# maxim2266/csvplus

Hardware: AMD Instinct MI355X
Metric: joined rows/sec (IndexOn build + chained Join, 1e8-row 3-col orders) (higher is better)
Workload: dtype u32; 1 GPU; BASELINE configs[3]: orders(1e8 x {cust_id,prod_id,qty}).Join(UniqueIndexOn customers.id 1e7).Join(UniqueIndexOn products.prod_id 1e5); rows=100000000, customers=10000000, products=100000, rows_this_rank=100000000, exchange=none (1 GPU), output=sorted positions

## Files before the change

csvplus_amd/csrc/chain.hip:

```cpp
#include <type_traits>

#include "probe_device.hpp"

namespace cph {

constexpr int kChainThreads = 256;
constexpr int kChainWaves   = kChainThreads / kWave;
constexpr int kChainRows    = 8;
constexpr int kWaveTile     = kWave * kChainRows;
constexpr int kChainTile    = kChainThreads * kChainRows;
constexpr int kChainMasks   = kChainRows * kChainWaves;
constexpr int kMaxChain     = 4;

struct ChainStepArg {
    DevCol col;
    const uint8_t* codec;
    const uint32_t* rowtab;
    const uint2* ranktab;
    int32_t positions;
    int32_t ranktab_lds;
    const uint4* hash;
    uint32_t hash_sectors;
    uint32_t hash_slice_mask;
    int32_t src;
    const uint32_t* src_perm;
    const void* codes;
    const uint32_t* perm;
    uint64_t n_index;
    int32_t codec_bytes;
    int32_t key32;
};
struct ChainArgs {
    ChainStepArg step[kMaxChain];
    uint32_t* out_rows[kMaxChain];
    int32_t nt_streams;
    int32_t reserved_;
};
struct LeanArgs {
    int32_t identity[kMaxChain];
    ArithPlan arith[kMaxChain];
};

template <int S, bool LONG, bool WIDE, bool DBG, uint32_t LEAN = 0, int R = kChainRows, bool DEP = false>
__global__ __launch_bounds__(kChainThreads) void k_chain_dense(ChainArgs a, uint64_t nprobe, uint64_t probe_base,
                                                              uint64_t ntiles, uint64_t* __restrict__ masks,
                                                              uint32_t* __restrict__ wave_counts, int dbg_flags, LeanArgs la) {
    extern __shared__ __attribute__((aligned(16))) uint8_t smem[];
    using B = std::conditional_t<WIDE, uint64_t, uint32_t>;
    using CW = std::conditional_t<WIDE, uint64_t, uint32_t>;
    const int dbg = DBG ? dbg_flags : 0;
    CodecView cv[S];
    {
        uint8_t* p = smem;
#pragma unroll
        for (int s = 0; s < S; s++) {
            if ((LEAN >> s) & 1u) continue;
            cv[s] = codec_load_to_lds(a.step[s].codec, p);
            p += a.step[s].codec_bytes;
        }
    }
    const CPH_LDS uint32_t* rank_lds[S];
    {
        uint8_t* p = smem;
#pragma unroll
        for (int s = 0; s < S; s++) p += a.step[s].codec_bytes;
        bool any = false;
#pragma unroll
        for (int s = 0; s < S; s++) {
            rank_lds[s] = nullptr;
            const int nblk = a.step[s].ranktab_lds;
            if (LEAN != 0 && nblk) {
                uint2* dst = reinterpret_cast<uint2*>(p);
                for (int i = threadIdx.x; i < 2 * nblk; i += kChainThreads) dst[i] = a.step[s].ranktab[i];
                rank_lds[s] = (const CPH_LDS uint32_t*)p;
                p += (size_t)nblk * 16;
                any = true;
            } else if (nblk) {
                uint32_t* dst = reinterpret_cast<uint32_t*>(p);
                for (int i = threadIdx.x; i < nblk; i += kChainThreads) {
                    const uint2 b0 = a.step[s].ranktab[2 * i], b1 = a.step[s].ranktab[2 * i + 1];
                    dst[3 * i] = b0.x;
                    dst[3 * i + 1] = b1.x;
                    dst[3 * i + 2] = b0.x ? b0.y : b1.y;
                }
                rank_lds[s] = (const CPH_LDS uint32_t*)p;
                p += (size_t)((nblk * 12 + 15) & ~15);
                any = true;
            }
        }
        if (any) __syncthreads();
    }
    const int lane = lane_id();
    const uint32_t wave = (uint32_t)__builtin_amdgcn_readfirstlane(wave_id());

#pragma unroll 1
    for (uint64_t tile = blockIdx.x; tile < ntiles; tile += gridDim.x) {
        uint32_t wave_matches = 0;
#pragma unroll 1
      for (int part = 0; part < kChainRows / R; part++) {
        const uint64_t wbase = tile * kChainTile + (uint64_t)wave * kWaveTile + (uint64_t)part * (R * kWave);
        const WaveRows<R> wr = wave_rows<R>(wbase, nprobe);
        uint32_t okm = wr.okm;
        WaveSpans<R, B> sp[S];
        uint64_t c0[S][R], c1[LONG ? S : 1][R];
        CW code[S][R];
        uint32_t brow[S][R];
#pragma unroll
      for (int lvl = 0; lvl < (DEP ? S : 1); lvl++) {
#pragma unroll
        for (int s = 0; s < S; s++) {
            if (DEP && s != lvl) continue;
            if ((LEAN >> s) & 1u) continue;
            if constexpr (DEP) {
                const int32_t src = a.step[s].src;
                if (src != 0) {
                    const int t = (src < 0 ? -src : src) - 1;
                    uint32_t grow[R];
#pragma unroll
                    for (int k = 0; k < R; k++) grow[k] = 0u;
#pragma unroll
                    for (int u = 0; u < S; u++)
                        if (u < s && u == t) {
#pragma unroll
                            for (int k = 0; k < R; k++) grow[k] = (okm >> k) & 1u ? brow[u][k] : 0u;
                        }
                    if (a.step[s].src_perm) {
#pragma unroll
                        for (int k = 0; k < R; k++) grow[k] = a.step[s].src_perm[grow[k]];
                    }
                    gather_spans<R, B>(a.step[s].col, grow, &sp[s]);
                    continue;
                }
            }
            if (a.nt_streams) wave_spans<R, B, false, true>(a.step[s].col, wr, &sp[s]);
            else wave_spans<R, B>(a.step[s].col, wr, &sp[s]);
        }
#pragma unroll
        for (int s = 0; s < S; s++) {
            if (DEP && s != lvl) continue;
            if ((LEAN >> s) & 1u) {
                typedef const __attribute__((address_space(1))) uint64_t* global_u64_ptr;
                const global_u64_ptr w = (global_u64_ptr)a.step[s].col.data + wr.rbase;
                if (a.nt_streams) {
#pragma unroll
                    for (int k = 0; k < R; k++) c0[s][k] = __builtin_nontemporal_load(&w[wr.rel[k]]);
                } else {
#pragma unroll
                    for (int k = 0; k < R; k++) c0[s][k] = w[wr.rel[k]];
                }
                continue;
            }
#pragma unroll
            for (int k = 0; k < R; k++) {
                c0[s][k] = a.nt_streams ? sp[s].chunk_nt(k, 0) : sp[s].chunk(k, 0);
                if constexpr (LONG) c1[s][k] = a.nt_streams ? sp[s].chunk_nt(k, 1) : sp[s].chunk(k, 1);
            }
        }
#pragma unroll
        for (int s = 0; s < S; s++) {
            if (DEP && s != lvl) continue;
            if (DBG && (dbg & 2)) {
#pragma unroll
                for (int k = 0; k < R; k++) code[s][k] = (CW)((c0[s][k] ^ (LONG ? c1[LONG ? s : 0][k] : 0ull)) & 1023);
            } else if ((LEAN >> s) & 1u) {
                encode_rows_arith<R, CW>(la.arith[s], c0[s], code[s], &okm);
            } else if (!WIDE || cv[s].hdr->lutw_bits == 32) {
                encode_rows<R, uint32_t, B, CW, LONG>(cv[s], sp[s], c0[s], c1[LONG ? s : 0], code[s], &okm,
                                                               a.step[s].col.fixed_width != 0 && (int)a.step[s].col.fixed_width == cv[s].hdr->col_maxlen[0]);
            } else {
                encode_rows<R, uint64_t, B, CW, LONG>(cv[s], sp[s], c0[s], c1[LONG ? s : 0], code[s], &okm,
                                                               a.step[s].col.fixed_width != 0 && (int)a.step[s].col.fixed_width == cv[s].hdr->col_maxlen[0]);
            }
        }
#pragma unroll
        for (int s = 0; s < S; s++) {
            if (DEP && s != lvl) continue;
            const ChainStepArg& st = a.step[s];
            if constexpr (LEAN != 0) {
                if (la.identity[s]) {
#pragma unroll
                    for (int k = 0; k < R; k++)
                        brow[s][k] = ((okm >> k) & 1u) && (uint32_t)code[s][k] < (uint32_t)st.n_index ? (uint32_t)code[s][k] : kTableAbsent;
                } else if (rank_lds[s]) {
#pragma unroll
                    for (int k = 0; k < R; k++) {
                        const uint32_t cidx = (okm >> k) & 1u ? (uint32_t)code[s][k] : 0u;
                        const CPH_LDS uint32_t* e = rank_lds[s] + 2u * (cidx >> 5);
                        const uint32_t bits = e[0], before = e[1], bit = cidx & 31u;
                        brow[s][k] = (bits >> bit) & 1u ? before + (uint32_t)__popc(bits & ((1u << bit) - 1u)) : kTableAbsent;
                    }
                } else {
                    uint2 blk[R];
#pragma unroll
                    for (int k = 0; k < R; k++) {
                        const uint32_t cidx = (okm >> k) & 1u ? (uint32_t)code[s][k] : 0u;
                        blk[k] = st.ranktab[cidx >> 5];
                    }
#pragma unroll
                    for (int k = 0; k < R; k++) {
                        const uint32_t bit = (uint32_t)code[s][k] & 31u;
                        brow[s][k] = (blk[k].x >> bit) & 1u ? blk[k].y + (uint32_t)__popc(blk[k].x & ((1u << bit) - 1u)) : kTableAbsent;
                    }
                }
            } else if (st.ranktab) {
                if (rank_lds[s]) {
#pragma unroll
                    for (int k = 0; k < R; k++) {
                        const CW cidx = (okm >> k) & 1u ? code[s][k] : (CW)0;
                        const CPH_LDS uint32_t* e = rank_lds[s] + 3u * (uint32_t)((uint64_t)cidx >> 6);
                        const uint32_t bit = (uint32_t)cidx & 63u;
                        const uint64_t bits = (uint64_t)e[0] | ((uint64_t)e[1] << 32);
                        const bool present = (bits >> bit) & 1ull;
                        brow[s][k] = present ? e[2] + (uint32_t)__popcll(bits & ((1ull << bit) - 1ull)) : kTableAbsent;
                    }
                } else {
                    uint2 blk[R];
#pragma unroll
                    for (int k = 0; k < R; k++) {
                        const CW cidx = (okm >> k) & 1u ? code[s][k] : (CW)0;
                        blk[k] = (DBG && (dbg & 1)) ? make_uint2(~0u, 0u) : st.ranktab[(uint64_t)cidx >> 5];
                    }
#pragma unroll
                    for (int k = 0; k < R; k++) {
                        const uint32_t bit = (uint32_t)code[s][k] & 31u;
                        const bool present = (blk[k].x >> bit) & 1u;
                        brow[s][k] = present ? blk[k].y + (uint32_t)__popc(blk[k].x & ((1u << bit) - 1u)) : kTableAbsent;
                    }
                }
            } else if (st.rowtab) {
#pragma unroll
                for (int k = 0; k < R; k++) {
                    const CW cidx = (okm >> k) & 1u ? code[s][k] : (CW)0;
                    brow[s][k] = (DBG && (dbg & 1)) ? 0u : st.rowtab[cidx];
                }
            } else if (st.hash) {
                const HashView hv{st.hash, st.hash_sectors, st.hash_slice_mask};
#pragma unroll
                for (int g = 0; g < R; g += 4) {
// ... 23 lines not shown
                    uint64_t lo;
                    bool hit;
                    if (st.key32) {
                        const uint32_t* cd = reinterpret_cast<const uint32_t*>(st.codes);
                        lo = lower_bound_dev<uint32_t>(cd, 0, st.n_index, (uint32_t)code[s][k]);
                        hit = lo < st.n_index && cd[lo] == (uint32_t)code[s][k];
                    } else {
                        const uint64_t* cd = reinterpret_cast<const uint64_t*>(st.codes);
                        lo = lower_bound_dev<uint64_t>(cd, 0, st.n_index, (uint64_t)code[s][k]);
                        hit = lo < st.n_index && cd[lo] == (uint64_t)code[s][k];
                    }
                    if (hit) brow[s][k] = st.positions ? (uint32_t)lo : st.perm[lo];
                }
            }
        }
#pragma unroll
        for (int s = 0; s < S; s++) {
            if (DEP && s != lvl) continue;
#pragma unroll
            for (int k = 0; k < R; k++)
                if (brow[s][k] == kTableAbsent) okm &= ~(1u << k);
        }
      }
        const uint64_t mword = (tile * kChainWaves + wave) * kChainRows + (uint64_t)part * R;
#pragma unroll
        for (int k = 0; k < R; k++) {
            const bool ok = (okm >> k) & 1u;
            const uint64_t bal = __ballot(ok);
            wave_matches += (uint32_t)__popcll(bal);
            if (lane == 0) masks[mword + k] = bal;
            if (ok && !(DBG && (dbg & 4))) {
#pragma unroll
                for (int s = 0; s < S; s++) {
                    if (a.nt_streams) __builtin_nontemporal_store(brow[s][k], a.out_rows[s] + wr.rbase + wr.rel[k]);
                    else (a.out_rows[s] + wr.rbase)[wr.rel[k]] = brow[s][k];
                }
            }
        }
      }
        if (lane == 0) wave_counts[tile * kChainWaves + wave] = wave_matches;
    }
}

struct CodeStepArg {
    const uint32_t* codes;
    const uint32_t* rowtab;
    const uint2* ranktab;
    uint64_t n_index, table_entries;
    int32_t identity;
    int32_t reserved_;
};
struct CodeArgs {
    CodeStepArg step[kMaxChain];
    uint32_t* out_rows[kMaxChain];
};
template <int S>
__global__ __launch_bounds__(kChainThreads) void k_chain_codes(CodeArgs a, uint64_t nprobe, uint64_t ntiles, uint64_t* __restrict__ masks,
                                                              uint32_t* __restrict__ wave_counts) {
    const int lane = lane_id();
    const uint32_t wave = (uint32_t)__builtin_amdgcn_readfirstlane(wave_id());
#pragma unroll 1
    for (uint64_t tile = blockIdx.x; tile < ntiles; tile += gridDim.x) {
        const uint64_t wbase = tile * kChainTile + (uint64_t)wave * kWaveTile;
        const WaveRows<kChainRows> wr = wave_rows<kChainRows>(wbase, nprobe);
        uint32_t okm = wr.okm;
        uint32_t code[S][kChainRows], brow[S][kChainRows];
#pragma unroll
// ... 265 lines not shown
    __shared__ uint32_t s_tmp[kPjThreads / kWave + 1];
    const uint64_t i0 = (uint64_t)blockIdx.x * kPjTile + (uint64_t)threadIdx.x * kPjItems;
    uint32_t keep = 0, mine = 0;
#pragma unroll
    for (int k = 0; k < kPjItems; k++)
        if (i0 + k < n && v[i0 + k] != kTableAbsent) {
            keep |= 1u << k;
            mine++;
        }
    uint32_t total;
    uint32_t run = block_exclusive_sum<uint32_t, kPjThreads>(mine, s_tmp, &total);
    uint64_t o = (uint64_t)tile_base[blockIdx.x] + run;
#pragma unroll
    for (int k = 0; k < kPjItems; k++) {
        if (!((keep >> k) & 1u)) continue;
        a.dst64[o] = a.src64[i0 + k];
        for (int j = 0; j < a.n32; j++) a.dst32[j][o] = a.src32[j][i0 + k];
        o++;
    }
}

bool chain_fast_path_ok(const ChainStep* steps, int nsteps) {
    if (nsteps > kMaxChain) return false;
    for (int s = 0; s < nsteps; s++) {
        const cph_index* ix = steps[s].index;
        if (steps[s].ncols != 1 || ix->nkeycols != 1) return false;
        if (ix->first_dup != UINT64_MAX) return false;
        if (ix->codec.nwords != 1 || ix->codec.npos == 0 || !ix->windows.empty()) return false;
        if (codec_premultiplied_bits(ix->codec) == 0) return false;
    }
    return true;
}

template <int S>
static Status enqueue_dense(cph_ctx* ctx, const ChainStep* steps, uint64_t nprobe, uint64_t probe_base,
                            uint32_t* const* d_rows, uint64_t* d_masks, uint32_t* d_counts, uint64_t* d_total,
                            ChainArgs* args_out, unsigned* grid_out, bool positions, uint64_t* host_total = nullptr,
                            const char* prof_name = "k_chain_dense") {
    const uint64_t ntiles = (nprobe + kChainTile - 1) / kChainTile;
    ChainArgs args{};
    LeanArgs largs{};
    size_t lds = 0, rank_lds_bytes = 0;
    const int dbg = ctx->chain_debug;
    bool long_keys = false, wide = false, dep = false;
    for (int s = 0; s < S; s++) dep |= steps[s].source != 0;
    if (dep) long_keys = wide = true;
    for (int s = 0; s < S; s++) {
        const cph_index* ix = steps[s].index;
        const DevCol& c = steps[s].cols[0];
        long_keys |= ix->codec.col_maxlen[0] > 8;
        wide |= codec_premultiplied_bits(ix->codec) != 32 || !ix->codec.key32;
        wide |= !col_is_narrow(c);
    }
    uint32_t lean = 0;
    bool ident[kMaxChain] = {false, false, false, false};
    if (positions)
        for (int s = 0; s < S; s++) {
            const cph_index* ix = steps[s].index;
            ident[s] = ctx->chain_identity && ix->table_entries != 0 && ix->table_entries == ix->nrows &&
                       ix->first_dup == UINT64_MAX && ix->windows.empty();
        }
    if (positions && ctx->chain_arith && !long_keys && !wide && !dbg) {
        bool all_ranked = true;
        for (int s = 0; s < S; s++) {
            const cph_index* ix = steps[s].index;
            const DevCol& c = steps[s].cols[0];
            ArithPlan ap;
            codec_arith_plan(ix->codec, &ap);
            if (ap.enabled && ap.keylen == 8 && c.fixed_width == 8 && ((uintptr_t)c.data & 7u) == 0) lean |= 1u << s;
            if (!ident[s]) {
                CPH_TRY(index_ensure_ranktab(ctx, ix));
                all_ranked &= (bool)ix->ranktab;
            }
        }
        if (!all_ranked) lean = 0;
    }
    if (S > 2 && lean != (1u << S) - 1u) lean = 0;
    if (!lean)
        for (int s = 0; s < S; s++) ident[s] = false;
    for (int s = 0; s < S; s++)
        if (!((lean >> s) & 1u)) lds += steps[s].index->codec_dev.bytes();
    for (int s = 0; s < S; s++) {
        const cph_index* ix = steps[s].index;
        ChainStepArg& st = args.step[s];
        st.col = steps[s].cols[0];
        st.codec = ix->codec_dev.as<uint8_t>();
        st.codec_bytes = (int32_t)ix->codec_dev.bytes();
        if ((lean >> s) & 1u) {
            codec_arith_plan(ix->codec, &largs.arith[s]);
            st.codec_bytes = 0;
        }
        st.positions = positions ? 1 : 0;
        st.rowtab = nullptr;
        st.ranktab = nullptr;
        largs.identity[s] = ident[s] ? 1 : 0;
        if (ident[s]) {
        } else if (positions) {
            CPH_TRY(index_ensure_ranktab(ctx, ix));
            st.ranktab = ix->ranktab ? ix->ranktab.as<uint2>() : nullptr;
            const size_t nblk = ranktab_blocks(ix->table_entries) / 2, rb = lean ? nblk * 16 : (nblk * 12 + 15) & ~(size_t)15;
            if (st.ranktab && ctx->chain_rank_lds && lds + rank_lds_bytes + rb <= 52 * 1024) {
                st.ranktab_lds = (int32_t)nblk;
                rank_lds_bytes += rb;
            }
        } else {
            CPH_TRY(index_ensure_rowtab(ctx, ix));
            st.rowtab = ix->rowtab ? ix->rowtab.as<uint32_t>() : nullptr;
        }
        st.src = steps[s].source;
        st.src_perm = (steps[s].source > 0 && positions) ? steps[steps[s].source - 1].index->perm.as<uint32_t>() : nullptr;
        st.hash = nullptr;
        st.hash_sectors = 0;
        st.hash_slice_mask = 0;
        if (!st.rowtab && !st.ranktab && !ident[s] && index_wants_hash(ix)) {
            CPH_TRY(index_ensure_hash(ctx, ix));
            if (ix->hash_mode == kHashK1) {
                st.hash = ix->hash.as<uint4>();
                st.hash_sectors = ix->hash_sectors;
                st.hash_slice_mask = ix->hash_slice_mask;
            }
        }
        st.codes = ix->sorted_codes.get();
        st.perm = ix->perm.as<uint32_t>();
        st.n_index = ix->nrows;
        st.key32 = ix->codec.key32 ? 1 : 0;
        args.out_rows[s] = d_rows[s];
    }
    lds += rank_lds_bytes;
    args.nt_streams = ctx->chain_nt_streams == 1 || (ctx->chain_nt_streams == 2 && positions) ? 1 : 0;
    const uint64_t ncounts = ntiles * kChainWaves;
    using KernelFn = void (*)(ChainArgs, uint64_t, uint64_t, uint64_t, uint64_t*, uint32_t*, int, LeanArgs);
    static const KernelFn variants[2][2][2] = {
        {{&k_chain_dense<S, false, false, false>, &k_chain_dense<S, false, false, true>},
         {&k_chain_dense<S, false, true, false>, &k_chain_dense<S, false, true, true>}},
        {{&k_chain_dense<S, true, false, false>, &k_chain_dense<S, true, false, true>},
         {&k_chain_dense<S, true, true, false>, &k_chain_dense<S, true, true, true>}}};
    KernelFn kernel = variants[long_keys ? 1 : 0][wide ? 1 : 0][(dbg && !dep) ? 1 : 0];
    if (!dbg && ctx->chain_rows4 != 0 && ((S == 2 && long_keys && wide) || (S >= 3 && (long_keys || wide)) || S == 4 || ctx->chain_rows4 == 2)) {
        static const KernelFn r4[2][2] = {{&k_chain_dense<S, false, false, false, 0u, 4>, &k_chain_dense<S, false, true, false, 0u, 4>},
                                          {&k_chain_dense<S, true, false, false, 0u, 4>, &k_chain_dense<S, true, true, false, 0u, 4>}};
        kernel = r4[long_keys ? 1 : 0][wide ? 1 : 0];
    }
    if constexpr (S >= 2) {
        if (dep) kernel = &k_chain_dense<S, true, true, false, 0u, 4, true>;
    }
    if (lean) {
        constexpr uint32_t kAll = (1u << S) - 1u;
        if (lean == kAll) kernel = &k_chain_dense<S, false, false, false, kAll>;
        if constexpr (S == 2) {
            if (lean == 1u) kernel = &k_chain_dense<S, false, false, false, 1u>;
            if (lean == 2u) kernel = &k_chain_dense<S, false, false, false, 2u>;
        }
    }
    int per_cu = 1, cus = 256;
    CPH_TRY(kernel_setup(ctx, reinterpret_cast<const void*>(kernel), kChainThreads, lds, &per_cu));
    CPH_TRY(device_cus(ctx, &cus));
    const unsigned grid = (unsigned)std::min<uint64_t>(ntiles, (uint64_t)cus * (uint64_t)per_cu);
    {
        ProfScope ps(ctx, prof_name, 0);
        hipLaunchKernelGGL(kernel, dim3(grid), dim3(kChainThreads), lds, ctx->stream, args, nprobe, probe_base,
                           ntiles, d_masks, d_counts, dep ? 0 : dbg, largs);
    }
    if (host_total) {
        DevBuf& acc = ctx->self_clean[ctx->stream_slot].sum;
        CPH_TRY(self_clean_block(ctx, &acc, 16));
        ProfScope ps(ctx, "k_sum_counts", 4.0 * (double)ncounts);
        const unsigned sgrid = sum_counts_grid(ncounts);
        hipLaunchKernelGGL(k_sum_counts_report, dim3(sgrid), dim3(256), 0, ctx->stream, d_counts, ncounts, acc.as<unsigned long long>(),
                           reinterpret_cast<unsigned long long*>(host_total));
    } else if (d_total) {
        ProfScope ps(ctx, "k_sum_counts", 4.0 * (double)ncounts);
        CPH_HIP_TRY(hipMemsetAsync(d_total, 0, sizeof(uint64_t), ctx->stream));
        const unsigned sgrid = (unsigned)std::min<uint64_t>((ncounts + 255) / 256, 512);
        hipLaunchKernelGGL(k_sum_counts, dim3(sgrid), dim3(256), 0, ctx->stream, d_counts, ncounts,
                           reinterpret_cast<unsigned long long*>(d_total));
    }
    CPH_HIP_TRY(hipGetLastError());
    if (args_out) *args_out = args;
    if (grid_out) *grid_out = grid;
    return {};
}

bool chain_fast_path_ok(const ChainStep* steps, int nsteps);

Status chain_enqueue_dense(cph_ctx* ctx, const ChainStep* steps, int nsteps, uint64_t nprobe, uint64_t probe_base,
                           uint32_t* const* d_rows, uint64_t* d_masks, uint32_t* d_counts, uint64_t* d_total, bool positions) {
// ... 368 lines not shown
```

csvplus_amd/csrc/codec_device.hpp:

```cpp
#pragma once

#include "cph_internal.hpp"
#include "device_utils.hpp"

namespace cph {

__device__ __forceinline__ uint64_t find_first_byte(const uint8_t* data, uint64_t begin, uint64_t len, uint32_t d) {
    const uint64_t dv = 0x0101010101010101ull * (uint64_t)(d & 0xFFu);
    for (uint64_t j = 0; 8 * j < len; j++) {
        const uint64_t x = load_value_chunk(data, begin, len, (int)j) ^ dv;
        const uint64_t t = (x - 0x0101010101010101ull) & ~x & 0x8080808080808080ull;
        if (t) {
            const uint64_t pos = 8 * j + (uint64_t)((__ffsll((long long)t) - 1) >> 3);
            return pos < len ? pos : len;
        }
    }
    return len;
}

__device__ __forceinline__ void value_span_whole(const DevCol& col, uint64_t row, uint64_t* begin, uint64_t* len);
__device__ __forceinline__ void value_span(const DevCol& col, uint64_t row, uint64_t* begin, uint64_t* len) {
    value_span_whole(col, row, begin, len);
    if (col.split) {
        const uint64_t b = *begin, l = *len;
// ... 135 lines not shown
        const uint32_t sym = (uint32_t)q < len ? ((uint32_t)(chunk >> (8 * (q & 7))) & 0xFFu) + 1u : 0u;
        const W v = lutw[q * kLutStride + sym];
        bad |= v;
        acc += v;
    }
    *code = (uint64_t)acc;
    return len <= (uint32_t)maxlen && !(bad >> (sizeof(W) * 8 - 1));
}

template <int R>
struct WaveRows {
    uint64_t rbase;
    uint32_t nvalid;
    uint32_t rel[R];
    uint32_t okm;
};
template <int R>
__device__ __forceinline__ WaveRows<R> wave_rows(uint64_t wbase, uint64_t nrows ) {
    WaveRows<R> w;
    const uint64_t left = nrows > wbase ? nrows - wbase : 0;
    w.nvalid = left > (uint64_t)(R * kWave) ? (uint32_t)(R * kWave) : (uint32_t)left;
    w.rbase = w.nvalid ? wbase : nrows - 1;
    const uint32_t rmax = w.nvalid ? w.nvalid - 1 : 0;
    w.okm = 0;
    const uint32_t lane = (uint32_t)lane_id();
#pragma unroll
    for (int k = 0; k < R; k++) {
        const uint32_t r = (uint32_t)k * kWave + lane;
        w.okm |= (r < w.nvalid ? 1u : 0u) << k;
        w.rel[k] = r < rmax ? r : rmax;
    }
    return w;
}

template <int R, class B>
struct WaveSpans {
    const uint8_t* base8;
    uint32_t delta;
    B x[R];
    uint32_t len[R];
    __device__ __forceinline__ uint64_t chunk(int k, uint32_t j) const {
        return load_chunk_nobranch<B>(base8, delta, x[k], len[k], j);
    }
    __device__ __forceinline__ uint64_t chunk_nt(int k, uint32_t j) const {
        return load_chunk_nobranch<B, true>(base8, delta, x[k], len[k], j);
    }
};
template <int R, class B, bool SEG = false, bool NT = false>
__device__ __forceinline__ void wave_spans(const DevCol& c, const WaveRows<R>& wr, WaveSpans<R, B>* sp);
template <int R, class B, bool NT = false>
__device__ __forceinline__ void wave_spans_whole(const DevCol& c, const WaveRows<R>& wr, WaveSpans<R, B>* sp);
template <int R, class B, bool SEG, bool NT>
__device__ __forceinline__ void wave_spans(const DevCol& c, const WaveRows<R>& wr, WaveSpans<R, B>* sp) {
    wave_spans_whole<R, B, NT>(c, wr, sp);
    if constexpr (SEG) {
#pragma unroll
        for (int k = 0; k < R; k++) {
            const uint32_t s = sp->len[k] < c.skip ? sp->len[k] : c.skip;
            sp->x[k] += (B)s;
            uint32_t l = sp->len[k] - s;
            if (c.take != 0xFFFFFFFFu && l > c.take) l = c.take;
            sp->len[k] = l;
        }
    }
}
template <int R, class B, bool NT>
// ... 134 lines not shown
        const int qn = maxlen - 8 * j < 8 ? maxlen - 8 * j : 8;
        const CPH_LDS W* lp = lutw + (8 * j) * kLutStride;
        if (fixed) {
#pragma unroll
            for (int b = 0; b < 8; b++)
                if (b < qn) encode_position<R, W, B, true>(lp, b, (uint32_t)(8 * j + b), sp, cur, acc, bad);
        } else {
#pragma unroll
            for (int b = 0; b < 8; b++)
                if (b < qn) encode_position<R, W, B, false>(lp, b, (uint32_t)(8 * j + b), sp, cur, acc, bad);
        }
    }
    uint32_t m = *okmask;
#pragma unroll
    for (int k = 0; k < R; k++) {
        code[k] = (CW)acc[k];
        const W flag = sizeof(W) == 4 ? acc[k] : bad[k];
        const bool good = sp.len[k] <= (uint32_t)maxlen && !(flag >> (sizeof(W) * 8 - 1));
        if (!good) m &= ~(1u << k);
    }
    *okmask = m;
}

struct ArithPlan {
    uint32_t enabled;
    uint32_t mul24;
    uint32_t keylen;
    uint32_t keep[2];
    uint32_t lo[2];
    uint32_t rngc[2];
    uint32_t wa[2], wb[2];
    uint32_t ma[2];
    uint32_t s1;
};

void codec_arith_plan(const CodecHost& codec, ArithPlan* ap);

template <int R, class CW>
__device__ __forceinline__ void encode_rows_arith(const ArithPlan& ap, const uint64_t (&c0)[R], CW (&code)[R], uint32_t* okmask) {
    uint32_t m = *okmask;
    uint32_t zl[R], zh[R];
#pragma unroll
    for (int k = 0; k < R; k++) {
        const uint32_t xl = (uint32_t)c0[k], xh = (uint32_t)(c0[k] >> 32);
        zl[k] = xl - ap.lo[0];
        zh[k] = xh - ap.lo[1];
        const uint32_t tl = zl[k] + ap.rngc[0], th = zh[k] + ap.rngc[1];
        const uint32_t bad = ((xl | zl[k] | tl) | (xh | zh[k] | th)) & 0x80808080u;
        if (bad) m &= ~(1u << k);
    }
    if (ap.mul24) {
#pragma unroll
        for (int k = 0; k < R; k++) {
            const uint32_t pa0 = __builtin_amdgcn_udot4(zl[k], ap.wa[0], 0u, false);
            const uint32_t pa1 = __builtin_amdgcn_udot4(zh[k], ap.wa[1], 0u, false);
            const uint32_t w0 = __builtin_amdgcn_udot4(zl[k], ap.wb[0], __umul24(pa0, ap.ma[0]), false);
            code[k] = (CW)__builtin_amdgcn_udot4(zh[k], ap.wb[1], __umul24(pa1, ap.ma[1]) + __umul24(w0, ap.s1), false);
        }
    } else {
#pragma unroll
        for (int k = 0; k < R; k++) {
            const uint32_t pa0 = __builtin_amdgcn_udot4(zl[k], ap.wa[0], 0u, false);
            const uint32_t pa1 = __builtin_amdgcn_udot4(zh[k], ap.wa[1], 0u, false);
            const uint32_t w0 = __builtin_amdgcn_udot4(zl[k], ap.wb[0], pa0 * ap.ma[0], false);
            code[k] = (CW)__builtin_amdgcn_udot4(zh[k], ap.wb[1], pa1 * ap.ma[1] + w0 * ap.s1, false);
        }
    }
    *okmask = m;
}

template <bool LONGV = true>
struct ValueHeadT {
    uint64_t begin = 0, len = 0, c0 = 0, c1 = 0, c2 = 0;
    __device__ __forceinline__ void span(const DevCol& col, uint64_t row) { value_span(col, row, &begin, &len); }
    __device__ __forceinline__ void chunks(const DevCol& col) {
        c0 = len > 0 ? load_value_chunk(col.data, begin, len, 0) : 0;
        c1 = len > 8 ? load_value_chunk(col.data, begin, len, 1) : 0;
        c2 = len > 16 ? load_value_chunk(col.data, begin, len, 2) : 0;
    }
    __device__ __forceinline__ void chunks_nobranch(const DevCol& col) {
        const uint64_t p = (uint64_t)(uintptr_t)col.data;
        const uint8_t* base8 = (const uint8_t*)(uintptr_t)(p & ~7ull);
        const uint32_t delta = (uint32_t)(p & 7ull);
        const uint32_t l32 = len > 0xFFFFFFFFull ? 0xFFFFFFFFu : (uint32_t)len;
        const uint64_t a = load_chunk_nobranch<uint64_t>(base8, delta, begin, l32, 0);
        const uint64_t b = load_chunk_nobranch<uint64_t>(base8, delta, begin, l32, 1);
        const uint64_t c = load_chunk_nobranch<uint64_t>(base8, delta, begin, l32, 2);
        c0 = l32 > 0 ? a : 0;
        c1 = l32 > 8 ? b : 0;
        c2 = l32 > 16 ? c : 0;
    }
    __device__ __forceinline__ void load(const DevCol& col, uint64_t row) {
        span(col, row);
        chunks(col);
    }
    __device__ __forceinline__ uint64_t chunk(const DevCol& col, int j) const {
        if constexpr (LONGV) {
            if (8ull * (uint64_t)j >= len) return 0;
            return j == 0 ? c0 : j == 1 ? c1 : j == 2 ? c2 : load_value_chunk(col.data, begin, len, j);
// ... 146 lines not shown
```

csvplus_amd/csrc/keycodec.hip:

```cpp
#include <algorithm>
#include <cmath>
#include <mutex>

#include "codec_device.hpp"
#include "host_encode_kernels.hpp"

namespace cph {

constexpr int kStatsThreads = 256;
constexpr int kStatsRows = 8;

template <class B, bool SEG>
__global__ __launch_bounds__(kStatsThreads) void k_col_stats(DevCol col, uint32_t* __restrict__ g_minmax,
                                                            uint32_t* __restrict__ g_mask) {
    __shared__ __attribute__((aligned(16))) uint8_t s_flag[kMaxKeyBytes * 256];
    __shared__ uint32_t s_min, s_max;
    {
        uint4* z = reinterpret_cast<uint4*>(s_flag);
        for (int i = threadIdx.x; i < kMaxKeyBytes * 256 / 16; i += kStatsThreads) z[i] = make_uint4(0, 0, 0, 0);
    }
    if (threadIdx.x == 0) { s_min = 0xFFFFFFFFu; s_max = 0; }
    __syncthreads();

    uint32_t mn = 0xFFFFFFFFu, mx = 0;
// ... 1597 lines not shown
                    else { dtags[k][h] = tag; dicts[k][h] = key; g.count++; }
                }
            }
        }
    }, 2048);
    const int best = split_pick(ctx, 0, cand, hs, step, most, plain_bits);
    if (best < 0) return {};
    const SplitStats& st = hs[(size_t)best];
    if (st.flags || st.count == 0 || st.count > (uint32_t)kWideDictMax || st.pmax > (uint32_t)kWideBytes || st.smax > (uint32_t)kSplitMaxSuffix ||
        st.vmax > (uint32_t)kSplitMaxValue)
        return {};
    std::vector<WideKey> dict;
    for (size_t s2 = 0; s2 < dtags[(size_t)best].size(); s2++)
        if (dtags[(size_t)best][s2]) dict.push_back(dicts[(size_t)best][s2]);
    if (dict.size() != st.count) return {};
    CodecHost trial;
    bool usable = false;
    CPH_TRY(split_assemble(ctx, 0, 1, nullptr, (uint32_t)cand[(size_t)best], st, &dict, plain_bits, &trial, &usable));
    if (!usable) return {};
    trial.spec_checked = true;
    if (trial.nwords != 1 || !trial.key32 || trial.word_states[0] > (1ull << 27)) return {};
    if (codec_sort_cost(trial) < bits_sort_cost(plain_bits)) *codec = std::move(trial);
    return {};
}

int codec_premultiplied_bits(const CodecHost& cd) {
    if (cd.nwords != 1 || cd.npos <= 0 || cd.has_groups()) return 0;
    const int bits = cd.word_states[0] <= (1ull << 31) ? 32 : 64;
    return (size_t)cd.npos * kLutStride * (size_t)(bits / 8) <= 48 * 1024 ? bits : 0;
}

void codec_arith_plan(const CodecHost& cd, ArithPlan* ap) {
    *ap = ArithPlan{};
    if (cd.ncols != 1 || cd.nwords != 1 || cd.has_groups() || cd.npos < 1 || cd.npos > 8) return;
    if (cd.col_minlen[0] != cd.col_maxlen[0] || cd.word_states[0] > (1ull << 31)) return;
    uint32_t lo[8] = {0}, rng[8] = {0}, radix[8] = {1, 1, 1, 1, 1, 1, 1, 1};
    for (int p = 0; p < cd.npos; p++) {
        const uint16_t* lut = &cd.lut[(size_t)p * kLutStride];
        if (lut[0] != kLutInvalid) return;
        int first = -1, last = -1, count = 0;
        for (int b = 0; b < 256; b++)
            if (lut[1 + b] != kLutInvalid) { if (first < 0) first = b; last = b; count++; }
        if (first < 0 || last >= 0x80 || last - first + 1 != count || count > 255 || count != (int)cd.radix[(size_t)p]) return;
        for (int b = first; b <= last; b++)
            if (lut[1 + b] != (uint16_t)(b - first)) return;
        lo[p] = (uint32_t)first;
        rng[p] = (uint32_t)(last - first);
        radix[p] = (uint32_t)count;
    }
    ap->keylen = (uint32_t)cd.npos;
    for (int w = 0; w < 2; w++) {
        for (int i = 0; i < 4; i++) {
            const int p = 4 * w + i;
            if (p < cd.npos) ap->keep[w] |= 0xFFu << (8 * i);
            ap->lo[w] |= lo[p] << (8 * i);
            ap->rngc[w] |= (0x7Fu - rng[p]) << (8 * i);
        }
        ap->wa[w] = radix[4 * w + 1] | 1u << 8;
        ap->wb[w] = radix[4 * w + 3] << 16 | 1u << 24;
        ap->ma[w] = radix[4 * w + 2] * radix[4 * w + 3];
    }
    const uint64_t s0 = (uint64_t)radix[0] * radix[1] * radix[2] * radix[3];
    const uint64_t s1 = (uint64_t)radix[4] * radix[5] * radix[6] * radix[7];
    ap->s1 = (uint32_t)s1;
    ap->mul24 = s0 <= (1ull << 24) && s1 < (1ull << 24) ? 1u : 0u;
    ap->enabled = 1;
}

Status codec_upload(cph_ctx* ctx, const CodecHost& cd, DevBuf* dev) {
    CodecDevHeader h{};
    h.ncols = cd.ncols;
    h.npos = cd.npos;
    h.nwords = cd.nwords;
    h.key32 = cd.key32 ? 1 : 0;
    for (int c = 0; c <= cd.ncols; c++) h.col_start[c] = cd.col_start[c];
    for (int c = cd.ncols + 1; c <= kMaxKeyCols; c++) h.col_start[c] = cd.npos;
    for (int c = 0; c < cd.ncols; c++) h.col_maxlen[c] = cd.col_maxlen[c];
    auto align16 = [](size_t x) { return (x + 15) & ~(size_t)15; };
    size_t off = align16(sizeof(CodecDevHeader));
    h.mult_off = (int32_t)off;
    off = align16(off + sizeof(uint64_t) * (size_t)cd.npos);
    h.wordof_off = (int32_t)off;
    off = align16(off + (size_t)cd.npos + 1);
    const int lutw_bits = codec_premultiplied_bits(cd);
    h.lutw_bits = lutw_bits;
    if (lutw_bits) {
        h.lut_off = 0;
        h.lutw_off = (int32_t)off;
        off = align16(off + (size_t)(lutw_bits / 8) * (size_t)cd.npos * kLutStride);
    } else {
        h.lutw_off = 0;
        h.lut_off = (int32_t)off;
        off = align16(off + sizeof(uint16_t) * (size_t)cd.npos * kLutStride);
    }
    if (cd.has_groups()) {
        h.ngroups = 0;
        for (int p = 0; p < cd.npos; p++) h.ngroups += cd.unit[(size_t)p] == kUnitHead || cd.unit[(size_t)p] == kUnitWide;
        h.unit_off = (int32_t)off;
        off = align16(off + (size_t)cd.npos);
// ... 584 lines not shown
```

Baseline: 149.0 billion rows/s.

## Add variable-length arithmetic lean path and compile-time switches for chain join kernel

```diff
diff --git a/csvplus_amd/csrc/chain.hip b/csvplus_amd/csrc/chain.hip
--- a/csvplus_amd/csrc/chain.hip
+++ b/csvplus_amd/csrc/chain.hip
@@ -41,13 +41,18 @@
     ArithPlan arith[kMaxChain];
 };
 
-template <int S, bool LONG, bool WIDE, bool DBG, uint32_t LEAN = 0, int R = kChainRows, bool DEP = false>
-__global__ __launch_bounds__(kChainThreads) void k_chain_dense(ChainArgs a, uint64_t nprobe, uint64_t probe_base,
+constexpr int kSwNt = 1, kSwMul24 = 2, kSwRuntime = 4;
+constexpr int chain_min_waves(int S, uint32_t lean) { return S <= 2 && lean == (1u << S) - 1u ? 4 : 1; }
+template <int S, bool LONG, bool WIDE, bool DBG, uint32_t LEAN = 0, int R = kChainRows, bool DEP = false, uint32_t VAR = 0, int SW = kSwRuntime>
+__global__ __launch_bounds__(kChainThreads, chain_min_waves(S, LEAN)) void k_chain_dense(ChainArgs a, uint64_t nprobe, uint64_t probe_base,
                                                               uint64_t ntiles, uint64_t* __restrict__ masks,
                                                               uint32_t* __restrict__ wave_counts, int dbg_flags, LeanArgs la) {
     extern __shared__ __attribute__((aligned(16))) uint8_t smem[];
     using B = std::conditional_t<WIDE, uint64_t, uint32_t>;
     using CW = std::conditional_t<WIDE, uint64_t, uint32_t>;
+    static_assert((VAR & ~LEAN) == 0 && (LEAN != 0 || SW == kSwRuntime), "VAR and SW describe lean steps");
+    constexpr int kM24 = (SW & kSwRuntime) ? -1 : ((SW & kSwMul24) ? 1 : 0);
+    const bool nt_streams = (SW & kSwRuntime) ? a.nt_streams != 0 : (SW & kSwNt) != 0;
     const int dbg = DBG ? dbg_flags : 0;
     CodecView cv[S];
     {
@@ -60,6 +65,7 @@
         }
     }
     const CPH_LDS uint32_t* rank_lds[S];
+    bool rank_in_lds[S];
     {
         uint8_t* p = smem;
 #pragma unroll
@@ -68,6 +74,7 @@
 #pragma unroll
         for (int s = 0; s < S; s++) {
             rank_lds[s] = nullptr;
+            rank_in_lds[s] = a.step[s].ranktab_lds != 0;
             const int nblk = a.step[s].ranktab_lds;
             if (LEAN != 0 && nblk) {
                 uint2* dst = reinterpret_cast<uint2*>(p);
@@ -92,6 +99,15 @@
     }
     const int lane = lane_id();
     const uint32_t wave = (uint32_t)__builtin_amdgcn_readfirstlane(wave_id());
+    uint64_t vend[S];
+#pragma unroll
+    for (int s = 0; s < S; s++) {
+        vend[s] = 0;
+        if ((VAR >> s) & 1u) {
+            const DevCol& c = a.step[s].col;
+            vend[s] = c.fixed_width ? nprobe * (uint64_t)c.fixed_width : (uint64_t)reinterpret_cast<const uint32_t*>(c.offsets)[nprobe];
+        }
+    }
 
 #pragma unroll 1
     for (uint64_t tile = blockIdx.x; tile < ntiles; tile += gridDim.x) {
@@ -99,17 +115,44 @@
 #pragma unroll 1
       for (int part = 0; part < kChainRows / R; part++) {
         const uint64_t wbase = tile * kChainTile + (uint64_t)wave * kWaveTile + (uint64_t)part * (R * kWave);
-        const WaveRows<R> wr = wave_rows<R>(wbase, nprobe);
+        const WaveRows<R> wr = LEAN != 0 ? wave_rows_full_first<R>(wbase, nprobe) : wave_rows<R>(wbase, nprobe);
         uint32_t okm = wr.okm;
         WaveSpans<R, B> sp[S];
         uint64_t c0[S][R], c1[LONG ? S : 1][R];
         CW code[S][R];
         uint32_t brow[S][R];
+        uint32_t vbeg[VAR ? S : 1][R], vstop[VAR ? S : 1][R], vlen[VAR ? S : 1][R];
+        uint64_t vbase[VAR ? S : 1], vlast[VAR ? S : 1];
 #pragma unroll
       for (int lvl = 0; lvl < (DEP ? S : 1); lvl++) {
 #pragma unroll
         for (int s = 0; s < S; s++) {
             if (DEP && s != lvl) continue;
+            if ((VAR >> s) & 1u) {
+                const DevCol& c = a.step[s].col;
+                if (c.fixed_width) {
+                    vbase[s] = wr.rbase * (uint64_t)c.fixed_width;
+#pragma unroll
+                    for (int k = 0; k < R; k++) {
+                        vbeg[s][k] = wr.rel[k] * c.fixed_width;
+                        vstop[s][k] = vbeg[s][k] + c.fixed_width;
+                    }
+                } else {
+                    typedef const __attribute__((address_space(1))) uint32_t* global_u32_ptr;
+                    const global_u32_ptr off = (global_u32_ptr) reinterpret_cast<const uint32_t*>(c.offsets) + wr.rbase;
+                    auto load_offsets = [&](auto nt) {
+#pragma unroll
+                        for (int k = 0; k < R; k++) {
+                            vbeg[s][k] = decltype(nt)::value ? __builtin_nontemporal_load(&off[wr.rel[k]]) : off[wr.rel[k]];
+                            vstop[s][k] = decltype(nt)::value ? __builtin_nontemporal_load(&off[wr.rel[k] + 1]) : off[wr.rel[k] + 1];
+                        }
+                    };
+                    if (nt_streams) load_offsets(std::true_type{});
+                    else load_offsets(std::false_type{});
+                    vbase[s] = 0;
+                }
+                continue;
+            }
             if ((LEAN >> s) & 1u) continue;
             if constexpr (DEP) {
                 const int32_t src = a.step[s].src;
@@ -132,16 +175,47 @@
                     continue;
                 }
             }
-            if (a.nt_streams) wave_spans<R, B, false, true>(a.step[s].col, wr, &sp[s]);
+            if (nt_streams) wave_spans<R, B, false, true>(a.step[s].col, wr, &sp[s]);
             else wave_spans<R, B>(a.step[s].col, wr, &sp[s]);
         }
+#pragma unroll
+        for (int pass = 0; pass < (VAR ? 2 : 1); pass++)
 #pragma unroll
         for (int s = 0; s < S; s++) {
             if (DEP && s != lvl) continue;
+            if ((int)((VAR >> s) & 1u) != pass) continue;
+            if ((VAR >> s) & 1u) {
+                const uint64_t p = (uint64_t)(uintptr_t)a.step[s].col.data + vbase[s];
+                vlast[s] = vbase[s] + (uint32_t)__builtin_amdgcn_readlane((int)vstop[s][R - 1], kWave - 1);
+#pragma unroll
+                for (int k = 0; k < R; k++) vlen[s][k] = vstop[s][k] - vbeg[s][k];
+                auto load_keys = [&](auto nt) {
+                    constexpr bool NT = decltype(nt)::value;
+                    if (vlast[s] + 8u <= vend[s]) {
+                        typedef const __attribute__((address_space(1))) uint8_t* global_u8_ptr;
+                        typedef uint64_t __attribute__((aligned(1))) u64_unaligned;
+                        typedef const __attribute__((address_space(1))) u64_unaligned* global_u64u_ptr;
+                        const global_u8_ptr b8 = (global_u8_ptr)(uintptr_t)p;
+#pragma unroll
+                        for (int k = 0; k < R; k++) {
+                            const global_u64u_ptr wp = (global_u64u_ptr)(b8 + vbeg[s][k]);
+                            c0[s][k] = NT ? __builtin_nontemporal_load(wp) : *wp;
+                        }
+                    } else {
+                        const uint8_t* base8 = (const uint8_t*)(uintptr_t)(p & ~7ull);
+                        const uint32_t delta = (uint32_t)(p & 7ull);
+#pragma unroll
+                        for (int k = 0; k < R; k++) c0[s][k] = load_chunk_nobranch<uint32_t, NT>(base8, delta, vbeg[s][k], vlen[s][k], 0);
+                    }
+                };
+                if (nt_streams) load_keys(std::true_type{});
+                else load_keys(std::false_type{});
+                continue;
+            }
             if ((LEAN >> s) & 1u) {
                 typedef const __attribute__((address_space(1))) uint64_t* global_u64_ptr;
                 const global_u64_ptr w = (global_u64_ptr)a.step[s].col.data + wr.rbase;
-                if (a.nt_streams) {
+                if (nt_streams) {
 #pragma unroll
                     for (int k = 0; k < R; k++) c0[s][k] = __builtin_nontemporal_load(&w[wr.rel[k]]);
                 } else {
@@ -152,8 +226,8 @@
             }
 #pragma unroll
             for (int k = 0; k < R; k++) {
-                c0[s][k] = a.nt_streams ? sp[s].chunk_nt(k, 0) : sp[s].chunk(k, 0);
-                if constexpr (LONG) c1[s][k] = a.nt_streams ? sp[s].chunk_nt(k, 1) : sp[s].chunk(k, 1);
+                c0[s][k] = nt_streams ? sp[s].chunk_nt(k, 0) : sp[s].chunk(k, 0);
+                if constexpr (LONG) c1[s][k] = nt_streams ? sp[s].chunk_nt(k, 1) : sp[s].chunk(k, 1);
             }
         }
 #pragma unroll
@@ -162,8 +236,10 @@
             if (DBG && (dbg & 2)) {
 #pragma unroll
                 for (int k = 0; k < R; k++) code[s][k] = (CW)((c0[s][k] ^ (LONG ? c1[LONG ? s : 0][k] : 0ull)) & 1023);
+            } else if ((VAR >> s) & 1u) {
+                encode_rows_arith_var<R, CW, kM24>(la.arith[s], c0[s], vlen[s], code[s], &okm);
             } else if ((LEAN >> s) & 1u) {
-                encode_rows_arith<R, CW>(la.arith[s], c0[s], code[s], &okm);
+                encode_rows_arith<R, CW, kM24>(la.arith[s], c0[s], code[s], &okm);
             } else if (!WIDE || cv[s].hdr->lutw_bits == 32) {
                 encode_rows<R, uint32_t, B, CW, LONG>(cv[s], sp[s], c0[s], c1[LONG ? s : 0], code[s], &okm,
                                                                a.step[s].col.fixed_width != 0 && (int)a.step[s].col.fixed_width == cv[s].hdr->col_maxlen[0]);
@@ -181,13 +257,18 @@
 #pragma unroll
                     for (int k = 0; k < R; k++)
                         brow[s][k] = ((okm >> k) & 1u) && (uint32_t)code[s][k] < (uint32_t)st.n_index ? (uint32_t)code[s][k] : kTableAbsent;
-                } else if (rank_lds[s]) {
+                } else if (rank_in_lds[s]) {
+                    uint64_t blk[R];
 #pragma unroll
                     for (int k = 0; k < R; k++) {
                         const uint32_t cidx = (okm >> k) & 1u ? (uint32_t)code[s][k] : 0u;
-                        const CPH_LDS uint32_t* e = rank_lds[s] + 2u * (cidx >> 5);
-                        const uint32_t bits = e[0], before = e[1], bit = cidx & 31u;
-                        brow[s][k] = (bits >> bit) & 1u ? before + (uint32_t)__popc(bits & ((1u << bit) - 1u)) : kTableAbsent;
+                        blk[k] = *(const CPH_LDS uint64_t*)(rank_lds[s] + 2u * (cidx >> 5));
+                    }
+#pragma unroll
+                    for (int k = 0; k < R; k++) {
+                        const uint32_t bits = (uint32_t)blk[k], before = (uint32_t)(blk[k] >> 32), bit = (uint32_t)code[s][k] & 31u;
+                        const uint32_t pos = before + (uint32_t)__popc(bits & ((1u << bit) - 1u));
+                        brow[s][k] = ((okm >> k) & 1u) && ((bits >> bit) & 1u) ? pos : kTableAbsent;
                     }
                 } else {
                     uint2 blk[R];
@@ -203,7 +284,7 @@
                     }
                 }
             } else if (st.ranktab) {
-                if (rank_lds[s]) {
+                if (rank_in_lds[s]) {
 #pragma unroll
                     for (int k = 0; k < R; k++) {
                         const CW cidx = (okm >> k) & 1u ? code[s][k] : (CW)0;
@@ -293,7 +374,7 @@
             if (ok && !(DBG && (dbg & 4))) {
 #pragma unroll
                 for (int s = 0; s < S; s++) {
-                    if (a.nt_streams) __builtin_nontemporal_store(brow[s][k], a.out_rows[s] + wr.rbase + wr.rel[k]);
+                    if (nt_streams) __builtin_nontemporal_store(brow[s][k], a.out_rows[s] + wr.rbase + wr.rel[k]);
                     else (a.out_rows[s] + wr.rbase)[wr.rel[k]] = brow[s][k];
                 }
             }
@@ -625,6 +706,20 @@
     return true;
 }
 
+using ChainKernelFn = void (*)(ChainArgs, uint64_t, uint64_t, uint64_t, uint64_t*, uint32_t*, int, LeanArgs);
+template <int S, uint32_t LEAN, uint32_t VAR>
+static ChainKernelFn lean_kernel(bool nt, bool mul24) {
+    if constexpr (S <= 2) {
+        static const ChainKernelFn k[4] = {&k_chain_dense<S, false, false, false, LEAN, kChainRows, false, VAR, 0>,
+                                           &k_chain_dense<S, false, false, false, LEAN, kChainRows, false, VAR, kSwNt>,
+                                           &k_chain_dense<S, false, false, false, LEAN, kChainRows, false, VAR, kSwMul24>,
+                                           &k_chain_dense<S, false, false, false, LEAN, kChainRows, false, VAR, kSwNt | kSwMul24>};
+        return k[(nt ? kSwNt : 0) | (mul24 ? kSwMul24 : 0)];
+    } else {
+        return &k_chain_dense<S, false, false, false, LEAN, kChainRows, false, VAR, kSwRuntime>;
+    }
+}
+
 template <int S>
 static Status enqueue_dense(cph_ctx* ctx, const ChainStep* steps, uint64_t nprobe, uint64_t probe_base,
                             uint32_t* const* d_rows, uint64_t* d_masks, uint32_t* d_counts, uint64_t* d_total,
@@ -645,7 +740,8 @@
         wide |= codec_premultiplied_bits(ix->codec) != 32 || !ix->codec.key32;
         wide |= !col_is_narrow(c);
     }
-    uint32_t lean = 0;
+    uint32_t lean = 0, var = 0;
+    bool mul24 = true;
     bool ident[kMaxChain] = {false, false, false, false};
     if (positions)
         for (int s = 0; s < S; s++) {
@@ -660,19 +756,60 @@
             const DevCol& c = steps[s].cols[0];
             ArithPlan ap;
             codec_arith_plan(ix->codec, &ap);
-            if (ap.enabled && ap.keylen == 8 && c.fixed_width == 8 && ((uintptr_t)c.data & 7u) == 0) lean |= 1u << s;
+            if (ap.enabled && ap.keylen == 8 && c.fixed_width == 8 && ((uintptr_t)c.data & 7u) == 0) {
+                lean |= 1u << s;
+                mul24 &= ap.mul24 != 0;
+            } else if (ap.var_enabled && !c.segmented() && !c.split && (c.fixed_width ? c.fixed_width <= 8 : c.offset_bits == 32)) {
+                var |= 1u << s;
+                mul24 &= ap.mul24 != 0;
+            }
             if (!ident[s]) {
                 CPH_TRY(index_ensure_ranktab(ctx, ix));
                 all_ranked &= (bool)ix->ranktab;
             }
         }
-        if (!all_ranked) lean = 0;
-    }
-    if (S > 2 && lean != (1u << S) - 1u) lean = 0;
+        if (!all_ranked) lean = var = 0;
+    }
+    constexpr uint32_t kAll = (1u << S) - 1u;
+    if ((lean | var) == kAll && (S <= 2 || var == 0 || var == kAll)) lean |= var;
+    else var = 0;
+    if (S > 2 && lean != kAll) lean = 0;
     if (!lean)
         for (int s = 0; s < S; s++) ident[s] = false;
     for (int s = 0; s < S; s++)
         if (!((lean >> s) & 1u)) lds += steps[s].index->codec_dev.bytes();
+    args.nt_streams = ctx->chain_nt_streams == 1 || (ctx->chain_nt_streams == 2 && positions) ? 1 : 0;
+    const uint64_t ncounts = ntiles * kChainWaves;
+    using KernelFn = ChainKernelFn;
+    static const KernelFn variants[2][2][2] = {
+        {{&k_chain_dense<S, false, false, false>, &k_chain_dense<S, false, false, true>},
+         {&k_chain_dense<S, false, true, false>, &k_chain_dense<S, false, true, true>}},
+        {{&k_chain_dense<S, true, false, false>, &k_chain_dense<S, true, false, true>},
+         {&k_chain_dense<S, true, true, false>, &k_chain_dense<S, true, true, true>}}};
+    KernelFn kernel = variants[long_keys ? 1 : 0][wide ? 1 : 0][(dbg && !dep) ? 1 : 0];
+    if (!dbg && ctx->chain_rows4 != 0 && ((S == 2 && long_keys && wide) || (S >= 3 && (long_keys || wide)) || S == 4 || ctx->chain_rows4 == 2)) {
+        static const KernelFn r4[2][2] = {{&k_chain_dense<S, false, false, false, 0u, 4>, &k_chain_dense<S, false, true, false, 0u, 4>},
+                                          {&k_chain_dense<S, true, false, false, 0u, 4>, &k_chain_dense<S, true, true, false, 0u, 4>}};
+        kernel = r4[long_keys ? 1 : 0][wide ? 1 : 0];
+    }
+    if constexpr (S >= 2) {
+        if (dep) kernel = &k_chain_dense<S, true, true, false, 0u, 4, true>;
+    }
+    if (lean) {
+        const bool nt = args.nt_streams != 0;
+        if (lean == kAll && var == 0) kernel = lean_kernel<S, kAll, 0u>(nt, mul24);
+        if (lean == kAll && var == kAll) kernel = lean_kernel<S, kAll, kAll>(nt, mul24);
+        if constexpr (S == 2) {
+            if (lean == kAll && var == 1u) kernel = lean_kernel<S, kAll, 1u>(nt, mul24);
+            if (lean == kAll && var == 2u) kernel = lean_kernel<S, kAll, 2u>(nt, mul24);
+            if (lean == 1u) kernel = lean_kernel<S, 1u, 0u>(nt, mul24);
+            if (lean == 2u) kernel = lean_kernel<S, 2u, 0u>(nt, mul24);
+        }
+    }
+    constexpr int kRankLdsGroups = 3;
+    constexpr size_t kMaxLdsPerGroup = 64 * 1024;
+    int per_cu_regs = 1;
+    CPH_TRY(kernel_setup(ctx, reinterpret_cast<const void*>(kernel), kChainThreads, lds, &per_cu_regs));
     for (int s = 0; s < S; s++) {
         const cph_index* ix = steps[s].index;
         ChainStepArg& st = args.step[s];
@@ -692,9 +829,13 @@
             CPH_TRY(index_ensure_ranktab(ctx, ix));
             st.ranktab = ix->ranktab ? ix->ranktab.as<uint2>() : nullptr;
             const size_t nblk = ranktab_blocks(ix->table_entries) / 2, rb = lean ? nblk * 16 : (nblk * 12 + 15) & ~(size_t)15;
-            if (st.ranktab && ctx->chain_rank_lds && lds + rank_lds_bytes + rb <= 52 * 1024) {
-                st.ranktab_lds = (int32_t)nblk;
-                rank_lds_bytes += rb;
+            if (st.ranktab && ctx->chain_rank_lds && lds + rank_lds_bytes + rb <= kMaxLdsPerGroup) {
+                int per_cu_with = 0;
+                CPH_TRY(kernel_setup(ctx, reinterpret_cast<const void*>(kernel), kChainThreads, lds + rank_lds_bytes + rb, &per_cu_with));
+                if (per_cu_with >= std::min(per_cu_regs, kRankLdsGroups)) {
+                    st.ranktab_lds = (int32_t)nblk;
+                    rank_lds_bytes += rb;
+                }
             }
         } else {
             CPH_TRY(index_ensure_rowtab(ctx, ix));
@@ -720,31 +861,6 @@
         args.out_rows[s] = d_rows[s];
     }
     lds += rank_lds_bytes;
-    args.nt_streams = ctx->chain_nt_streams == 1 || (ctx->chain_nt_streams == 2 && positions) ? 1 : 0;
-    const uint64_t ncounts = ntiles * kChainWaves;
-    using KernelFn = void (*)(ChainArgs, uint64_t, uint64_t, uint64_t, uint64_t*, uint32_t*, int, LeanArgs);
-    static const KernelFn variants[2][2][2] = {
-        {{&k_chain_dense<S, false, false, false>, &k_chain_dense<S, false, false, true>},
-         {&k_chain_dense<S, false, true, false>, &k_chain_dense<S, false, true, true>}},
-        {{&k_chain_dense<S, true, false, false>, &k_chain_dense<S, true, false, true>},
-         {&k_chain_dense<S, true, true, false>, &k_chain_dense<S, true, true, true>}}};
-    KernelFn kernel = variants[long_keys ? 1 : 0][wide ? 1 : 0][(dbg && !dep) ? 1 : 0];
-    if (!dbg && ctx->chain_rows4 != 0 && ((S == 2 && long_keys && wide) || (S >= 3 && (long_keys || wide)) || S == 4 || ctx->chain_rows4 == 2)) {
-        static const KernelFn r4[2][2] = {{&k_chain_dense<S, false, false, false, 0u, 4>, &k_chain_dense<S, false, true, false, 0u, 4>},
-                                          {&k_chain_dense<S, true, false, false, 0u, 4>, &k_chain_dense<S, true, true, false, 0u, 4>}};
-        kernel = r4[long_keys ? 1 : 0][wide ? 1 : 0];
-    }
-    if constexpr (S >= 2) {
-        if (dep) kernel = &k_chain_dense<S, true, true, false, 0u, 4, true>;
-    }
-    if (lean) {
-        constexpr uint32_t kAll = (1u << S) - 1u;
-        if (lean == kAll) kernel = &k_chain_dense<S, false, false, false, kAll>;
-        if constexpr (S == 2) {
-            if (lean == 1u) kernel = &k_chain_dense<S, false, false, false, 1u>;
-            if (lean == 2u) kernel = &k_chain_dense<S, false, false, false, 2u>;
-        }
-    }
     int per_cu = 1, cus = 256;
     CPH_TRY(kernel_setup(ctx, reinterpret_cast<const void*>(kernel), kChainThreads, lds, &per_cu));
     CPH_TRY(device_cus(ctx, &cus));
diff --git a/csvplus_amd/csrc/codec_device.hpp b/csvplus_amd/csrc/codec_device.hpp
--- a/csvplus_amd/csrc/codec_device.hpp
+++ b/csvplus_amd/csrc/codec_device.hpp
@@ -191,6 +191,20 @@
     }
     return w;
 }
+template <int R>
+__device__ __forceinline__ WaveRows<R> wave_rows_full_first(uint64_t wbase, uint64_t nrows ) {
+    if (nrows >= wbase + (uint64_t)(R * kWave)) {
+        WaveRows<R> w;
+        w.rbase = wbase;
+        w.nvalid = (uint32_t)(R * kWave);
+        w.okm = (1u << R) - 1u;
+        const uint32_t lane = (uint32_t)lane_id();
+#pragma unroll
+        for (int k = 0; k < R; k++) w.rel[k] = (uint32_t)k * kWave + lane;
+        return w;
+    }
+    return wave_rows<R>(wbase, nrows);
+}
 
 template <int R, class B>
 struct WaveSpans {
@@ -391,11 +405,27 @@
     uint32_t wa[2], wb[2];
     uint32_t ma[2];
     uint32_t s1;
+    uint32_t var_enabled;
+    uint32_t minlen;
+    uint32_t lenspan;
+    uint32_t padin[2];
 };
 
 void codec_arith_plan(const CodecHost& codec, ArithPlan* ap);
 
-template <int R, class CW>
+template <int M24>
+__device__ __forceinline__ uint32_t arith_dot(const ArithPlan& ap, uint32_t zl, uint32_t zh) {
+    const uint32_t pa0 = __builtin_amdgcn_udot4(zl, ap.wa[0], 0u, false);
+    const uint32_t pa1 = __builtin_amdgcn_udot4(zh, ap.wa[1], 0u, false);
+    if constexpr (M24 != 0) {
+        const uint32_t w0 = __builtin_amdgcn_udot4(zl, ap.wb[0], __umul24(pa0, ap.ma[0]), false);
+        return __builtin_amdgcn_udot4(zh, ap.wb[1], __umul24(pa1, ap.ma[1]) + __umul24(w0, ap.s1), false);
+    } else {
+        const uint32_t w0 = __builtin_amdgcn_udot4(zl, ap.wb[0], pa0 * ap.ma[0], false);
+        return __builtin_amdgcn_udot4(zh, ap.wb[1], pa1 * ap.ma[1] + w0 * ap.s1, false);
+    }
+}
+template <int R, class CW, int M24 = -1>
 __device__ __forceinline__ void encode_rows_arith(const ArithPlan& ap, const uint64_t (&c0)[R], CW (&code)[R], uint32_t* okmask) {
     uint32_t m = *okmask;
     uint32_t zl[R], zh[R];
@@ -408,22 +438,40 @@
         const uint32_t bad = ((xl | zl[k] | tl) | (xh | zh[k] | th)) & 0x80808080u;
         if (bad) m &= ~(1u << k);
     }
-    if (ap.mul24) {
-#pragma unroll
-        for (int k = 0; k < R; k++) {
-            const uint32_t pa0 = __builtin_amdgcn_udot4(zl[k], ap.wa[0], 0u, false);
-            const uint32_t pa1 = __builtin_amdgcn_udot4(zh[k], ap.wa[1], 0u, false);
-            const uint32_t w0 = __builtin_amdgcn_udot4(zl[k], ap.wb[0], __umul24(pa0, ap.ma[0]), false);
-            code[k] = (CW)__builtin_amdgcn_udot4(zh[k], ap.wb[1], __umul24(pa1, ap.ma[1]) + __umul24(w0, ap.s1), false);
-        }
+    if (M24 < 0 ? ap.mul24 != 0 : M24 != 0) {
+#pragma unroll
+        for (int k = 0; k < R; k++) code[k] = (CW)arith_dot<1>(ap, zl[k], zh[k]);
     } else {
 #pragma unroll
-        for (int k = 0; k < R; k++) {
-            const uint32_t pa0 = __builtin_amdgcn_udot4(zl[k], ap.wa[0], 0u, false);
-            const uint32_t pa1 = __builtin_amdgcn_udot4(zh[k], ap.wa[1], 0u, false);
-            const uint32_t w0 = __builtin_amdgcn_udot4(zl[k], ap.wb[0], pa0 * ap.ma[0], false);
-            code[k] = (CW)__builtin_amdgcn_udot4(zh[k], ap.wb[1], pa1 * ap.ma[1] + w0 * ap.s1, false);
-        }
+        for (int k = 0; k < R; k++) code[k] = (CW)arith_dot<0>(ap, zl[k], zh[k]);
+    }
+    *okmask = m;
+}
+
+template <int R, class CW, int M24 = -1>
+__device__ __forceinline__ void encode_rows_arith_var(const ArithPlan& ap, const uint64_t (&c0)[R], const uint32_t (&len)[R], CW (&code)[R],
+                                                      uint32_t* okmask) {
+    uint32_t m = *okmask;
+    uint32_t rl[R], rh[R];
+#pragma unroll
+    for (int k = 0; k < R; k++) {
+        const uint32_t sh = (len[k] < 8u ? len[k] : 8u) << 2;
+        const uint64_t past = (~0ull << sh) << sh;
+        const uint32_t pl = (uint32_t)past, ph = (uint32_t)(past >> 32);
+        const uint32_t xl = (pl & ap.lo[0]) | (~pl & (uint32_t)c0[k]), xh = (ph & ap.lo[1]) | (~ph & (uint32_t)(c0[k] >> 32));
+        const uint32_t zl = xl - ap.lo[0], zh = xh - ap.lo[1];
+        const uint32_t tl = zl + ap.rngc[0], th = zh + ap.rngc[1];
+        const uint32_t bad = ((xl | zl | tl) | (xh | zh | th)) & 0x80808080u;
+        if (bad != 0u || len[k] - ap.minlen > ap.lenspan) m &= ~(1u << k);
+        rl[k] = zl + (~pl & ap.padin[0]);
+        rh[k] = zh + (~ph & ap.padin[1]);
+    }
+    if (M24 < 0 ? ap.mul24 != 0 : M24 != 0) {
+#pragma unroll
+        for (int k = 0; k < R; k++) code[k] = (CW)arith_dot<1>(ap, rl[k], rh[k]);
+    } else {
+#pragma unroll
+        for (int k = 0; k < R; k++) code[k] = (CW)arith_dot<0>(ap, rl[k], rh[k]);
     }
     *okmask = m;
 }
diff --git a/csvplus_amd/csrc/keycodec.hip b/csvplus_amd/csrc/keycodec.hip
--- a/csvplus_amd/csrc/keycodec.hip
+++ b/csvplus_amd/csrc/keycodec.hip
@@ -1653,29 +1653,37 @@
 
 void codec_arith_plan(const CodecHost& cd, ArithPlan* ap) {
     *ap = ArithPlan{};
-    if (cd.ncols != 1 || cd.nwords != 1 || cd.has_groups() || cd.npos < 1 || cd.npos > 8) return;
-    if (cd.col_minlen[0] != cd.col_maxlen[0] || cd.word_states[0] > (1ull << 31)) return;
-    uint32_t lo[8] = {0}, rng[8] = {0}, radix[8] = {1, 1, 1, 1, 1, 1, 1, 1};
+    if (cd.ncols != 1 || cd.nwords != 1 || cd.has_groups() || cd.has_split() || cd.npos < 1 || cd.npos > 8) return;
+    if (cd.col_maxlen[0] != cd.npos || cd.col_minlen[0] < 0 || cd.col_minlen[0] > cd.col_maxlen[0] || cd.word_states[0] > (1ull << 31)) return;
+    const int minlen = cd.col_minlen[0];
+    uint32_t lo[8] = {0}, rng[8] = {0}, pad[8] = {0}, radix[8] = {1, 1, 1, 1, 1, 1, 1, 1};
     for (int p = 0; p < cd.npos; p++) {
         const uint16_t* lut = &cd.lut[(size_t)p * kLutStride];
-        if (lut[0] != kLutInvalid) return;
+        const bool padin = lut[0] != kLutInvalid;
+        if (padin != (p >= minlen) || (padin && lut[0] != 0)) return;
         int first = -1, last = -1, count = 0;
         for (int b = 0; b < 256; b++)
             if (lut[1 + b] != kLutInvalid) { if (first < 0) first = b; last = b; count++; }
-        if (first < 0 || last >= 0x80 || last - first + 1 != count || count > 255 || count != (int)cd.radix[(size_t)p]) return;
+        if (first < 0 || last >= 0x80 || last - first + 1 != count || count + (padin ? 1 : 0) > 255 ||
+            count + (padin ? 1 : 0) != (int)cd.radix[(size_t)p])
+            return;
         for (int b = first; b <= last; b++)
-            if (lut[1 + b] != (uint16_t)(b - first)) return;
+            if (lut[1 + b] != (uint16_t)(b - first + (padin ? 1 : 0))) return;
         lo[p] = (uint32_t)first;
         rng[p] = (uint32_t)(last - first);
-        radix[p] = (uint32_t)count;
-    }
-    ap->keylen = (uint32_t)cd.npos;
+        pad[p] = padin ? 1u : 0u;
+        radix[p] = (uint32_t)count + pad[p];
+    }
+    ap->minlen = (uint32_t)minlen;
+    ap->lenspan = (uint32_t)(cd.npos - minlen);
+    if (minlen == cd.npos) ap->keylen = (uint32_t)cd.npos;
     for (int w = 0; w < 2; w++) {
         for (int i = 0; i < 4; i++) {
             const int p = 4 * w + i;
             if (p < cd.npos) ap->keep[w] |= 0xFFu << (8 * i);
             ap->lo[w] |= lo[p] << (8 * i);
             ap->rngc[w] |= (0x7Fu - rng[p]) << (8 * i);
+            ap->padin[w] |= pad[p] << (8 * i);
         }
         ap->wa[w] = radix[4 * w + 1] | 1u << 8;
         ap->wb[w] = radix[4 * w + 3] << 16 | 1u << 24;
@@ -1685,7 +1693,8 @@
     const uint64_t s1 = (uint64_t)radix[4] * radix[5] * radix[6] * radix[7];
     ap->s1 = (uint32_t)s1;
     ap->mul24 = s0 <= (1ull << 24) && s1 < (1ull << 24) ? 1u : 0u;
-    ap->enabled = 1;
+    ap->var_enabled = 1;
+    ap->enabled = minlen == cd.npos ? 1 : 0;
 }
 
 Status codec_upload(cph_ctx* ctx, const CodecHost& cd, DevBuf* dev) {
```

Result: faster. 152.4 billion rows/s (median of 6 runs) (+2.3%).
